# AIGeeksGroup/UniVid

Hardware: AMD Instinct MI355X
Metric: denoise_steps_per_sec (higher is better)
Workload: dtype bf16

## Files before the change

### include/univid_hip.h

```cpp
#ifndef UNIVID_HIP_H
#define UNIVID_HIP_H
#include <stdint.h>
#ifdef __cplusplus
extern "C" {
#endif

int uv_version(void);
const char* uv_build_id(void);
int uv_init(void);
const char* uv_last_error(void);
int uv_device_arch(char* buf, int len);
int uv_host_blocking_sync(int on);

#define UV_OPT_CONV_HALO 0
#define UV_OPT_GEMM_GM 1
#define UV_OPT_ATTN_CUT 2
int uv_set_option(int key, int value);
int uv_get_option(int key, int* value);
int uv_reset_options(void);

#define UV_EPI_BF16 0
#define UV_EPI_GELU_BF16 1
#define UV_EPI_F32_FROM_BF16 2
#define UV_EPI_RESID_F32 3
#define UV_EPI_GATE_RESID_F32 4
#define UV_EPI_BF16_T 5

int uv_gemm_bf16_nt(const void* A, long lda, const void* W, long ldw, const void* bias_bf16, int M, int N, int K,
                    int epilogue, void* out, long ldo, const float* gate, const int32_t* gate_tid, long gate_stride,
                    int tile_cfg, void* stream);

int uv_gemm_bf16_nt_ws(const void* A, long lda, const void* W, long ldw, const void* bias_bf16, int M, int N, int K,
                       int epilogue, void* out, long ldo, const float* gate, const int32_t* gate_tid, long gate_stride,
                       int tile_cfg, void* workspace, long workspace_bytes, void* stream);
long uv_gemm_splitk_ws_bytes(int M, int N, int K);

int uv_gemm_f16_nt(const void* A, long lda, const void* W, long ldw, const void* bias_f16, int M, int N, int K, int epilogue,
                   void* out, long ldo, const float* gate, const int32_t* gate_tid, long gate_stride, int tile_cfg, void* stream);

int uv_gemm_bf16_nt_ssq(const void* A, long lda, const void* W, long ldw, const void* bias_bf16, int M, int N, int K, void* out, long ldo,
                        float* ssq, long ld_ssq, int tile_cfg, void* stream);
int uv_rms_scale_from_ssq(const float* ssq, long ld_ssq, int M, int groups, int C, float eps, float* rs, void* stream);

int uv_lora_down_bf16(const void* x, long ldx, const void* A, long lda, const float* scale, int M, int K, int R, void* out, long ldo,
                      int Rpad, void* stream);


int uv_mx_quant_bf16(const void* x, long ldx, void* codes, long ldc, void* scales, long ld_s, int M, int K, void* stream);

int uv_gemm_mxfp8_nt(const void* A, long lda, const void* A_scale, long ld_as, const void* W, long ldw, const void* W_scale, long ld_ws,
                     const void* bias_bf16, int M, int N, int K, int epilogue, void* out, long ldo, const float* gate,
                     const int32_t* gate_tid, long gate_stride, void* stream);

int uv_gemm_f32_nt(const float* A, long lda, const float* W, long ldw, const float* bias, int M, int N, int K, float* out,
                   long ldo, const float* resid, long ldr, void* stream);

int uv_flash_attn_bf16(const void* q, long ldq, const void* k, long ldk, const void* vt, long ldvt, void* out, long ldo,
                       int batch, int Lq, int Lk, int H, int head_dim, float softmax_scale, void* stream);

int uv_flash_attn_bf16_qnorm(const void* q, long ldq, const void* k, long ldk, const void* vt, long ldvt, void* out, long ldo,
                             int batch, int Lq, int Lk, int H, int head_dim, float softmax_scale, const float* q_rs, const float* q_weight,
                             void* stream);

int uv_flash_attn_f16(const void* q, long ldq, const void* k, long ldk, const void* vt, long ldvt, void* out, long ldo,
                      int batch, int Lq, int Lk, int H, int head_dim, float softmax_scale, void* stream);

int uv_flash_attn_kernel_name(int Lk, int head_dim, long ldk, long ldvt, int f16, char* buf, int len);

// ... 81 lines not shown
```

### univid_amd/_lib.py

```python
import ctypes
import os

import torch

_HERE = os.path.dirname(os.path.abspath(__file__))
LIB_PATH = os.path.join(_HERE, "libunivid_hip.so")

_c = ctypes
_P, _L, _I, _F = _c.c_void_p, _c.c_long, _c.c_int, _c.c_float

SIGNATURES = {
    "uv_version": [],
    "uv_init": [],
    "uv_last_error": [],
    "uv_build_id": [],
    "uv_device_arch": [_c.c_char_p, _I],
    "uv_host_blocking_sync": [_I],
    "uv_set_option": [_I, _I],
    "uv_get_option": [_I, _c.POINTER(_I)],
    "uv_reset_options": [],
    "uv_gemm_bf16_nt": [_P, _L, _P, _L, _P, _I, _I, _I, _I, _P, _L, _P, _P, _L, _I, _P],
    "uv_gemm_bf16_nt_ws": [_P, _L, _P, _L, _P, _I, _I, _I, _I, _P, _L, _P, _P, _L, _I, _P, _L, _P],
    "uv_gemm_splitk_ws_bytes": [_I, _I, _I],
    "uv_gemm_f16_nt": [_P, _L, _P, _L, _P, _I, _I, _I, _I, _P, _L, _P, _P, _L, _I, _P],
    "uv_mx_quant_bf16": [_P, _L, _P, _L, _P, _L, _I, _I, _P],
    "uv_gemm_mxfp8_nt": [_P, _L, _P, _L, _P, _L, _P, _L, _P, _I, _I, _I, _I, _P, _L, _P, _P, _L, _P],
    "uv_gemm_f32_nt": [_P, _L, _P, _L, _P, _I, _I, _I, _P, _L, _P, _L, _P],
    "uv_gemm_bf16_nt_ssq": [_P, _L, _P, _L, _P, _I, _I, _I, _P, _L, _P, _L, _I, _P],
    "uv_rms_scale_from_ssq": [_P, _L, _I, _I, _I, _F, _P, _P],
    "uv_lora_down_bf16": [_P, _L, _P, _L, _P, _I, _I, _I, _P, _L, _I, _P],
    "uv_cast_f32_bf16_rows": [_P, _L, _P, _L, _I, _I, _P],
    "uv_flash_attn_bf16_qnorm": [_P, _L, _P, _L, _P, _L, _P, _L, _I, _I, _I, _I, _I, _F, _P, _P, _P],
    "uv_flash_attn_bf16": [_P, _L, _P, _L, _P, _L, _P, _L, _I, _I, _I, _I, _I, _F, _P],
    "uv_flash_attn_f16": [_P, _L, _P, _L, _P, _L, _P, _L, _I, _I, _I, _I, _I, _F, _P],
    "uv_flash_attn_kernel_name": [_I, _I, _L, _L, _I, _c.c_char_p, _I],
    "uv_flash_attn_plan": [_I, _I, _I, _I, _I, _L, _L, _I, _c.c_char_p, _I, _c.POINTER(_I), _c.POINTER(_I), _c.POINTER(_I)],
    "uv_transpose_16": [_P, _L, _P, _L, _I, _I, _I, _P],
    "uv_cast_f32_to16": [_P, _P, _L, _I, _P],
    "uv_cast_16_to_f32": [_P, _P, _L, _I, _P],
    "uv_layernorm_mod": [_P, _L, _P, _L, _I, _I, _F, _I, _P, _L, _I, _I, _P, _P, _P, _I, _I, _P],
    "uv_t5_attention_bf16": [_P, _L, _P, _L, _P, _L, _P, _L, _I, _I, _P, _I, _P],
    "uv_add_bf16": [_P, _P, _P, _L, _P],
    "uv_t5_gated_gelu_bf16": [_P, _P, _P, _L, _P],
    "uv_gelu_erf_bf16": [_P, _P, _L, _P],
    "uv_interp_linear_rows_bf16": [_P, _L, _P, _L, _I, _I, _I, _P],
    "uv_l2_normalize_rows_f32": [_P, _L, _P, _L, _I, _I, _F, _P],
    "uv_rmsnorm_rope": [_P, _L, _P, _L, _P, _I, _I, _I, _F, _P, _I, _I, _I, _I, _P],
    "uv_rmsnorm_rope_qk": [_P, _P, _P, _P, _P, _P, _L, _L, _I, _I, _I, _I, _F, _P, _I, _I, _I, _I, _P],
    "uv_patchify_bf16": [_P, _P, _L, _I, _I, _I, _I, _I, _I, _I, _I, _P],
    "uv_unpatchify_f32": [_P, _L, _P, _I, _I, _I, _I, _I, _I, _I, _P],
    "uv_sinusoid_f32": [_P, _P, _I, _I, _P],
    "uv_linear_rows_f32": [_P, _L, _P, _P, _P, _L, _I, _I, _I, _I, _P],
    "uv_add_rows_f32": [_P, _P, _P, _I, _L, _P],
    "uv_cast_f32_bf16": [_P, _P, _L, _P],
    "uv_add_bf16_resid": [_P, _L, _P, _L, _I, _I, _P],
    "uv_text_weight_rows_bf16": [_P, _L, _P, _L, _I, _I, _I, _F, _P],
# ... 178 lines not shown
def host_blocking_sync(on=True, device=None):
    dev = torch.device("cuda" if device is None else device)
    idx = torch.cuda.current_device() if dev.index is None else dev.index
    lib = load()
    with torch.cuda.device(idx):
        if lib.uv_host_blocking_sync(1 if on else 0) != 0:
            raise UnividHipError(lib.uv_last_error().decode())


def gemm_splitk_ws_bytes(M, N, K, device=None):
    dev = torch.device("cuda" if device is None else device)
    idx = torch.cuda.current_device() if dev.index is None else dev.index
    lib = init(idx)
    with torch.cuda.device(idx):
        return int(lib.uv_gemm_splitk_ws_bytes(int(M), int(N), int(K)))


def gemm_bf16(a, w, bias, out, epi, M=None, gate=None, gate_tid=None, tile_cfg=0, ws=None):
    f16 = a.dtype == torch.float16
    _chk(a, torch.float16 if f16 else torch.bfloat16, "gemm_bf16.a")
    _chk(w, a.dtype, "gemm_bf16.w")
    M = a.shape[0] if M is None else M
    N, K = w.shape
    if ws is not None and not f16:
        _chk(ws, torch.uint8, "gemm_bf16.ws")
        call("uv_gemm_bf16_nt_ws", ptr(a), a.stride(0), ptr(w), w.stride(0), ptr(bias), M, N, K, epi, ptr(out), out.stride(0),
             ptr(gate), ptr(gate_tid), 0 if gate is None else gate.stride(0), tile_cfg, ptr(ws), ws.numel(), stream_ptr(), flops=2 * M * N * K)
        return out
    call("uv_gemm_f16_nt" if f16 else "uv_gemm_bf16_nt", ptr(a), a.stride(0), ptr(w), w.stride(0), ptr(bias), M, N, K, epi, ptr(out), out.stride(0),
         ptr(gate), ptr(gate_tid), 0 if gate is None else gate.stride(0), tile_cfg, stream_ptr(), flops=2 * M * N * K)
    return out


def mx_quant(x, codes, scales, M=None, K=None):
    _chk(x, torch.bfloat16, "mx_quant.x")
    _chk(codes, torch.uint8, "mx_quant.codes")
    _chk(scales, torch.uint8, "mx_quant.scales")
    M = x.shape[0] if M is None else M
    K = x.shape[1] if K is None else K
    if x.dim() != 2 or codes.dim() != 2 or scales.dim() != 2 or M > min(x.shape[0], codes.shape[0], scales.shape[0]) or \
            K > min(x.shape[1], codes.shape[1]) or K > 32 * scales.shape[1]:
        raise UnividHipError(f"mx_quant: x {tuple(x.shape)} / codes {tuple(codes.shape)} / scales {tuple(scales.shape)} do not fit M = {M}, K = {K}")
    call("uv_mx_quant_bf16", ptr(x), x.stride(0), ptr(codes), codes.stride(0), ptr(scales), scales.stride(0), M, K, stream_ptr())
    return codes, scales


def gemm_mxfp8(a, a_scale, w, w_scale, bias, out, epi, M=None, gate=None, gate_tid=None):
    for t, n in ((a, "a"), (a_scale, "a_scale"), (w, "w"), (w_scale, "w_scale")):
        _chk(t, torch.uint8, "gemm_mxfp8." + n)
    if bias is not None:
        _chk(bias, torch.bfloat16, "gemm_mxfp8.bias")
    M = a.shape[0] if M is None else M
    N, K = w.shape
    if a.shape[1] < K or M > min(a.shape[0], a_scale.shape[0]) or a_scale.shape[1] * 32 < K or w_scale.shape[1] * 32 < K or w_scale.shape[0] < N:
        raise UnividHipError(f"gemm_mxfp8: a {tuple(a.shape)} / a_scale {tuple(a_scale.shape)} / w {tuple(w.shape)} / w_scale "
                             f"{tuple(w_scale.shape)} do not fit M = {M}")
    call("uv_gemm_mxfp8_nt", ptr(a), a.stride(0), ptr(a_scale), a_scale.stride(0), ptr(w), w.stride(0), ptr(w_scale), w_scale.stride(0),
         ptr(bias), M, N, K, epi, ptr(out), out.stride(0), ptr(gate), ptr(gate_tid), 0 if gate is None else gate.stride(0), stream_ptr(),
         flops=2 * M * N * K)
    return out


def gemm_bf16_ssq(a, w, bias, out, ssq, M=None, tile_cfg=0):
    _chk(a, torch.bfloat16, "gemm_bf16_ssq.a")
    _chk(w, torch.bfloat16, "gemm_bf16_ssq.w")
    _chk(ssq, torch.float32, "gemm_bf16_ssq.ssq")
# ... 118 lines not shown
```

### univid_amd/csrc/gemm_bf16.hip

```cpp
#include "gemm_bf16_kernels.h"
#include <limits.h>

int uv_gemm_diag_launch(const GemmArgs& a, int epilogue, int tile_cfg, hipStream_t s);

struct GemmWs { void* p = nullptr; long bytes = 0; };

enum GemmKernel {
    GK_PERSIST,
    GK_PINGPONG,
    GK_RING128,
    GK_T128,
    GK_T256,
    GK_T256x192,
    GK_SPLITK4,
    GK_SPLITK2,
    GK_DIAG,
};
struct GemmStep { GemmKernel kernel; int m0, rows; };
struct GemmPlan { int n; GemmStep step[2]; };

static long whole_rounds_cut(int M, int N, int ncus) {
    const long tiles_n = (N + 255) / 256, tiles_m = (M + 255) / 256;
    const long rounds = tiles_m * tiles_n / ncus;
    return rounds * ncus / tiles_n * 256;
// ... 113 lines not shown
    UV_CHECK_ARG(a.zeros, "uv_gemm_bf16_nt: zero page missing (call uv_init)");
    const GemmPlan plan = plan_gemm(M, N, K, epilogue, ldo, tile_cfg, F16, uv_num_cus(), ws.p ? ws.bytes : 0, ((uintptr_t)ws.p & 255) == 0);
    for (int i = 0; i < plan.n; ++i) {
        const GemmStep& st = plan.step[i];
        const int rc = launch_step<F16>(st.kernel, rows_of(a, epilogue, st.m0, st.rows), epilogue, tile_cfg, (hipStream_t)stream, ws);
        if (rc) return rc;
    }
    return 0;
}

extern "C" int uv_gemm_bf16_nt(const void* A, long lda, const void* W, long ldw, const void* bias_bf16,
                               int M, int N, int K, int epilogue, void* out, long ldo,
                               const float* gate, const int32_t* gate_tid, long gate_stride,
                               int tile_cfg, void* stream) {
    return gemm_entry<false>(A, lda, W, ldw, bias_bf16, M, N, K, epilogue, out, ldo, gate, gate_tid, gate_stride, tile_cfg, stream);
}

extern "C" int uv_gemm_bf16_nt_ws(const void* A, long lda, const void* W, long ldw, const void* bias_bf16,
                                  int M, int N, int K, int epilogue, void* out, long ldo,
                                  const float* gate, const int32_t* gate_tid, long gate_stride,
                                  int tile_cfg, void* workspace, long workspace_bytes, void* stream) {
    UV_CHECK_ARG(workspace_bytes >= 0 && (workspace || workspace_bytes == 0), "uv_gemm_bf16_nt_ws: bad workspace");
    GemmWs ws;
    ws.p = workspace; ws.bytes = workspace_bytes;
    return gemm_entry<false>(A, lda, W, ldw, bias_bf16, M, N, K, epilogue, out, ldo, gate, gate_tid, gate_stride, tile_cfg, stream, nullptr, 0, ws);
}

extern "C" long uv_gemm_splitk_ws_bytes(int M, int N, int K) {
    const GemmPlan plan = plan_gemm(M, N, K, UV_EPI_RESID_F32, N, 0, false, uv_num_cus(), LONG_MAX, true);
    const GemmStep& strip = plan.step[plan.n - 1];
    return strip.kernel == GK_SPLITK4 ? splitk_ws_bytes(strip.rows, N, 4) : 0;
}

extern "C" int uv_gemm_bf16_nt_ssq(const void* A, long lda, const void* W, long ldw, const void* bias_bf16, int M, int N, int K,
                                   void* out, long ldo, float* ssq, long ld_ssq, int tile_cfg, void* stream) {
    return gemm_entry<false>(A, lda, W, ldw, bias_bf16, M, N, K, UV_EPI_BF16_SSQ, out, ldo, nullptr, nullptr, 0, tile_cfg, stream, ssq, ld_ssq);
}

extern "C" int uv_gemm_f16_nt(const void* A, long lda, const void* W, long ldw, const void* bias_f16,
                              int M, int N, int K, int epilogue, void* out, long ldo,
                              const float* gate, const int32_t* gate_tid, long gate_stride,
                              int tile_cfg, void* stream) {
    UV_CHECK_ARG(tile_cfg == 0, "uv_gemm_f16_nt: only tile_cfg 0 (automatic) is built for fp16 operands");
    return gemm_entry<true>(A, lda, W, ldw, bias_f16, M, N, K, epilogue, out, ldo, gate, gate_tid, gate_stride, tile_cfg, stream);
}
```

### univid_amd/csrc/gemm_bf16_kernels.h

```cpp
#pragma once
#include "common.h"
#include <stdlib.h>
#include <type_traits>

const float* uv_zero_page();

#define UV_BK 64

enum {
    UV_EPI_BF16 = 0,
    UV_EPI_GELU_BF16 = 1,
    UV_EPI_F32_FROM_BF16 = 2,
    UV_EPI_RESID_F32 = 3,
    UV_EPI_GATE_RESID_F32 = 4,
    UV_EPI_BF16_T = 5,
    UV_EPI_BF16_SSQ = 6,
};

struct GemmArgs {
    const bf16_t* A;
    const bf16_t* W;
    const bf16_t* bias;
    void* out;
    const float* gate;
// ... 836 lines not shown
            for (int hm = 0; hm < 2; ++hm)
#pragma unroll
                for (int j = 0; j < 4; ++j)
#pragma unroll
                    for (int hn = 0; hn < 2; ++hn)
                        epi_pair16<EPI, F16>(p, m0 + hm * 128 + wr * 64 + j * 16, n0 + hn * 128 + wc * 32, acc[hn][hm][0][j], acc[hn][hm][1][j], frow, fq);
        } else if constexpr (EPI == UV_EPI_BF16_T) {
#pragma unroll
            for (int hm = 0; hm < 2; ++hm)
#pragma unroll
                for (int j = 0; j < 4; j += 2)
#pragma unroll
                    for (int hn = 0; hn < 2; ++hn)
#pragma unroll
                        for (int i = 0; i < 2; ++i)
                            epi_pair16_T<F16>(p, m0 + hm * 128 + wr * 64 + j * 16, n0 + hn * 128 + wc * 32 + i * 16, acc[hn][hm][i][j], acc[hn][hm][i][j + 1], frow, fq);
        } else {
#pragma unroll
            for (int hm = 0; hm < 2; ++hm)
#pragma unroll
                for (int j = 0; j < 4; ++j)
#pragma unroll
                    for (int hn = 0; hn < 2; ++hn)
#pragma unroll
                        for (int i = 0; i < 2; ++i)
                            epi_frag<EPI, F16, true>(p, m0 + hm * 128 + wr * 64 + j * 16, n0 + hn * 128 + wc * 32 + i * 16, acc[hn][hm][i][j], frow, fq);
        }
        if (!has_next) break;
        m0 = m1; n0 = n1; cur = nxt;
    }
    asm volatile("s_waitcnt vmcnt(0)" ::: "memory");
}


template <void (*KERN)(GemmArgs)>
static int launch_kernel(dim3 grid, dim3 block, size_t lds, hipStream_t stream, const GemmArgs& a, const char* who) {
    UV_ONCE_PER_DEVICE(hipFuncSetAttribute((const void*)KERN, hipFuncAttributeMaxDynamicSharedMemorySize, (int)lds));
    hipLaunchKernelGGL(KERN, grid, block, lds, stream, a);
    UV_CHECK_LAUNCH(who);
    return 0;
}

constexpr unsigned UV_EPIS_ALL = 0x7f;
constexpr bool epi_in(unsigned epis, int e) { return e >= 0 && e < 32 && (epis >> e & 1) != 0; }
template <int E>
using epi_c = std::integral_constant<int, E>;
template <unsigned EPIS = UV_EPIS_ALL, class Launch>
static int launch_epi(int epi, Launch&& launch) {
    switch (epi) {
        case UV_EPI_BF16: if constexpr (epi_in(EPIS, UV_EPI_BF16)) return launch(epi_c<UV_EPI_BF16>()); break;
        case UV_EPI_GELU_BF16: if constexpr (epi_in(EPIS, UV_EPI_GELU_BF16)) return launch(epi_c<UV_EPI_GELU_BF16>()); break;
        case UV_EPI_F32_FROM_BF16: if constexpr (epi_in(EPIS, UV_EPI_F32_FROM_BF16)) return launch(epi_c<UV_EPI_F32_FROM_BF16>()); break;
        case UV_EPI_RESID_F32: if constexpr (epi_in(EPIS, UV_EPI_RESID_F32)) return launch(epi_c<UV_EPI_RESID_F32>()); break;
        case UV_EPI_GATE_RESID_F32: if constexpr (epi_in(EPIS, UV_EPI_GATE_RESID_F32)) return launch(epi_c<UV_EPI_GATE_RESID_F32>()); break;
        case UV_EPI_BF16_T: if constexpr (epi_in(EPIS, UV_EPI_BF16_T)) return launch(epi_c<UV_EPI_BF16_T>()); break;
        case UV_EPI_BF16_SSQ: if constexpr (epi_in(EPIS, UV_EPI_BF16_SSQ)) return launch(epi_c<UV_EPI_BF16_SSQ>()); break;
    }
    uv_set_error("uv_gemm_bf16_nt: unknown epilogue %d", epi);
    return -1;
}

template <int VAR = 0, bool F16 = false>
static int launch_8ph(const GemmArgs& a0, int epi, hipStream_t stream) {
    GemmArgs a = a0;
    a.tiles_m = (a.M + 255) / 256;
    a.tiles_n = (a.N + 255) / 256;
// ... 20 lines not shown
                 "uv_gemm_bf16_nt_ws: the split-K strip is built for the bf16 and the residual epilogues (0, 3, 4), not %d", epi);
    a.ws_cnt = (int*)ws;
    a.ws_slab = (float*)((char*)ws + 4096);
    if (hipMemsetAsync(a.ws_cnt, 0, (size_t)tiles * sizeof(int), stream) != hipSuccess) {
        uv_set_error("uv_gemm_bf16_nt_ws: hipMemsetAsync of the tile counters failed");
        return -1;
    }
    const dim3 grid(8 * ((tiles * SK + 7) / 8));
    return launch_epi<EPIS>(epi, [&](auto e) {
        return launch_kernel<gemm_bf16_8ph_kernel<decltype(e)::value, 5, F16, SK>>(grid, 512, 128 * 1024, stream, a, "uv_gemm_bf16_nt_ws");
    });
}

template <bool F16 = false>
static int launch_8ph_persist(const GemmArgs& a0, int epi, hipStream_t stream) {
    GemmArgs a = a0;
    UV_CHECK_ARG(a.M % 256 == 0 && a.N % 256 == 0, "uv_gemm_bf16_nt: the persistent kernel needs whole 256x256 tiles (M=%d N=%d)", a.M, a.N);
    UV_CHECK_ARG(a.ldo % 8 == 0 || (epi != UV_EPI_BF16_T && epi != UV_EPI_BF16 && epi != UV_EPI_GELU_BF16 && epi != UV_EPI_BF16_SSQ),
                 "uv_gemm_bf16_nt: the persistent kernel stores 16 bytes per lane: ldo=%ld must be a multiple of 8 elements", a.ldo);
    a.tiles_m = a.M / 256;
    a.tiles_n = a.N / 256;
    a.gm = (a.N <= 4096 && a.K <= 4096) ? 8 : (a.K >= 8192 ? 2 : 4);
    if (const int gm = uv_option(UV_OPT_GEMM_GM); gm > 0) a.gm = gm;
    const int tiles = a.tiles_m * a.tiles_n;
    int wgs = uv_num_cus() & ~7;
    if (wgs > tiles) wgs = tiles & ~7;
    UV_CHECK_ARG(wgs >= 8, "uv_gemm_bf16_nt: too few tiles (%d) for the persistent kernel", tiles);
    const dim3 grid(wgs);
    return launch_epi(epi, [&](auto e) {
        return launch_kernel<gemm_bf16_8ph_persist_kernel<decltype(e)::value, F16>>(grid, 512, 128 * 1024, stream, a, "uv_gemm_bf16_nt");
    });
}

template <int BM, int BN, int WM, int WN, int NS = 2, bool F16 = false>
static int launch_cfg(const GemmArgs& a0, int epi, hipStream_t stream) {
    GemmArgs a = a0;
    a.tiles_m = (a.M + BM - 1) / BM;
    a.tiles_n = (a.N + BN - 1) / BN;
    constexpr bool SSQ = (BN / WN) % 32 == 0;
    UV_CHECK_ARG(SSQ || epi != UV_EPI_BF16_SSQ, "uv_gemm_bf16_nt_ssq: this tile shape has no whole 32-column groups per wave");
    const dim3 grid(a.tiles_m * a.tiles_n);
    return launch_epi<SSQ ? UV_EPIS_ALL : UV_EPIS_ALL & ~(1u << UV_EPI_BF16_SSQ)>(epi, [&](auto e) {
        return launch_kernel<gemm_bf16_nt_kernel<BM, BN, WM, WN, decltype(e)::value, NS, F16>>(grid, WM * WN * 64, NS * (BM + BN) * 128, stream, a, "uv_gemm_bf16_nt");
    });
}
```

### univid_amd/wan/model.py

```python
import contextlib
import math
from typing import List, Optional

import torch
import torch.nn as nn

from .. import _lib
from .._lib import (EPI_BF16, EPI_BF16_T, EPI_F32_FROM_BF16, EPI_GATE_RESID_F32, EPI_GELU_BF16, EPI_RESID_F32)

__all__ = ["WanModel"]

BF16 = torch.bfloat16


def _round_up(x, m):
    return (x + m - 1) // m * m


def rope_params(max_seq_len, dim, theta=10000):
    ang = torch.outer(torch.arange(max_seq_len),
                      1.0 / torch.pow(theta, torch.arange(0, dim, 2).to(torch.float64).div(dim)))
    return torch.polar(torch.ones_like(ang), ang)


# ... 36 lines not shown
    if mode == "mxfp8":
        if dim % 256 or ffn_dim % 256:
            raise ValueError(f"ffn_precision 'mxfp8' needs dim and ffn_dim to be multiples of 256 (dim {dim}, ffn_dim {ffn_dim}): "
                             "uv_gemm_mxfp8_nt takes N % 256 == 0 and K % 128 == 0")
        if any(getattr(ffn[i], "_uv_lora", None) for i in (0, 2)):
            raise NotImplementedError(
                "ffn_precision 'mxfp8' and an un-merged LoRA adapter (merge=False) on ffn.0 / ffn.2 cannot be combined: the MXFP8 GEMM has no "
                "adapter slot. Detach the adapter or merge it (merge=True: the merged weights are re-quantised), or keep ffn_precision 'bf16'. "
                "Un-merged adapters on the attention projections work in both modes.")


LORA_MAX_SLOT = 512


class _LoraSlot:
    __slots__ = ("A", "scale", "S", "rows")

    def __init__(self, entries, dev):
        self.rows = [(ad, ad["A"].shape[0]) for ad in entries]
        R = sum(r for _, r in self.rows)
        self.S = _round_up(R, 128)
        if self.S > LORA_MAX_SLOT:
            raise ValueError(f"the adapters on the projections of one input stack to rank {R}: more than the {LORA_MAX_SLOT} slot columns "
                             f"(LORA_MAX_SLOT) an activation buffer carries")
        self.A = torch.cat([ad["A"].to(device=dev, dtype=BF16) for ad in entries]).contiguous()
        self.scale = torch.empty(R, dtype=torch.float32, device=dev)
        self.refresh_scale()

    def refresh_scale(self):
        host = torch.cat([torch.full((r,), float(ad["scaling"]) * float(ad["weight"]), dtype=torch.float32) for ad, r in self.rows])
        self.scale.copy_(host)


def _prepare_group(lins):
    preps = {n: _Prepared(l) for n, l in lins.items()}
    entries = [(n, ad) for n, l in lins.items() for ad in getattr(l, "_uv_lora", {}).values()]
    if not entries:
        return preps, None
    first = next(iter(preps.values())).w
    K, dev = first.shape[1], first.device
    slot = _LoraSlot([ad for _, ad in entries], dev)
    col = K
    for n, ad in entries:
        p, r = preps[n], ad["A"].shape[0]
        if p.w.shape[1] == K:
            w = torch.zeros(p.w.shape[0], K + slot.S, dtype=BF16, device=dev)
            w[:, :K] = p.w
            p.w = w
        p.w[:, col:col + r] = ad["B"].to(device=dev, dtype=BF16)
        col += r
    return preps, slot


def _act_buf(rows, K, slots, dev):
    S = max((s.S for s in slots if s is not None), default=0)
    return torch.empty(rows, K + S, dtype=BF16, device=dev)


def _slotted(t, K, slot, M=None):
    if slot is None:
        return t
    M = t.shape[0] if M is None else M
    if t.shape[1] < K + slot.S:
        e = torch.empty(t.shape[0], K + slot.S, dtype=BF16, device=t.device)
        e[:M, :K].copy_(t[:M, :K])
        t = e
    if M:
# ... 2 lines not shown


class WanRMSNorm(nn.Module):
    def __init__(self, dim, eps=1e-5):
        super().__init__()
        self.dim, self.eps = dim, eps
        self.weight = nn.Parameter(torch.ones(dim))


class WanLayerNorm(nn.LayerNorm):
    def __init__(self, dim, eps=1e-6, elementwise_affine=False):
        super().__init__(dim, elementwise_affine=elementwise_affine, eps=eps)


class WanSelfAttention(nn.Module):
    def __init__(self, dim, num_heads, window_size=(-1, -1), qk_norm=True, eps=1e-6):
        assert dim % num_heads == 0
        super().__init__()
        self.dim, self.num_heads, self.head_dim = dim, num_heads, dim // num_heads
        self.window_size, self.qk_norm, self.eps = window_size, qk_norm, eps
        if tuple(window_size) != (-1, -1) or not qk_norm:
            raise NotImplementedError("only the TI2V-5B setting (global attention, qk_norm) is built")
        self.q = nn.Linear(dim, dim)
        self.k = nn.Linear(dim, dim)
        self.v = nn.Linear(dim, dim)
        self.o = nn.Linear(dim, dim)
        self.norm_q = WanRMSNorm(dim, eps=eps)
        self.norm_k = WanRMSNorm(dim, eps=eps)
        self._prep = None
        self._slots = {}
        self._kv_cache = {}

    _groups = {"qkv": ("q", "k", "v"), "o": ("o",)}

    def prepare(self):
        self._prep, self._slots = {}, {}
        for g, names in self._groups.items():
            preps, self._slots[g] = _prepare_group({n: getattr(self, n) for n in names})
            self._prep.update(preps)
        self._kv_cache = {}

    def _self_attn(self, h, L, grid, freqs, x_resid, gate, gate_tid, batch=1, sp=None):
        if sp is not None:
            return self._self_attn_sp(h, L, grid, freqs, x_resid, gate, gate_tid, batch, sp)
        C, H, D = self.dim, self.num_heads, self.head_dim
        p = self._prep
        dev = h.device
        M = batch * L
        h = _slotted(h, C, self._slots["qkv"], M)
        ql = torch.empty(M, C, dtype=BF16, device=dev)
        kl = torch.empty(M, C, dtype=BF16, device=dev)
        vt = _vt_scratch("vt", C, batch, L, dev)
        _lib.gemm_bf16(h, p["q"].w, p["q"].b, ql, EPI_BF16, M=M)
        _lib.gemm_bf16(h, p["k"].w, p["k"].b, kl, EPI_BF16, M=M)
        _lib.gemm_bf16(h, p["v"].w, p["v"].b, vt, EPI_BF16_T, M=M)
        _lib.rmsnorm_rope_qk(ql, kl, self.norm_q.weight, self.norm_k.weight, M, L, C, D, self.eps, freqs, grid)
        att = _act_buf(M, C, (self._slots["o"],), dev)
        _lib.flash_attn(ql, kl, vt, att, L, L, H, D, 1.0 / math.sqrt(D), batch=batch)
        att = _slotted(att, C, self._slots["o"], M)
        _lib.gemm_bf16(att, p["o"].w, p["o"].b, x_resid, EPI_GATE_RESID_F32, M=M, gate=gate, gate_tid=gate_tid)

    def _self_attn_sp(self, h, n, grid, freqs, x_resid, gate, gate_tid, batch, sp):
        par, Lt, r0 = sp
        C, H, D = self.dim, self.num_heads, self.head_dim
        P = par.size
        if H % P or Lt % 8:
            raise NotImplementedError(f"sequence parallel needs heads % ranks == 0 and tokens % 8 == 0 (H={H}, p={P}, L={Lt})")
        p = self._prep
        dev = h.device
        M = batch * n
        Cp, Hp = C // P, H // P
        ql = torch.empty(M, C, dtype=BF16, device=dev)
        kl = torch.empty(M, C, dtype=BF16, device=dev)
        vt = torch.zeros(C, _round_up(max(M, 1), 64), dtype=BF16, device=dev)
        qf = torch.empty(batch * Lt, Cp, dtype=BF16, device=dev)
        kf = torch.empty(batch * Lt, Cp, dtype=BF16, device=dev)
        vtf = _vt_scratch("vt_sp", Cp, batch, Lt, dev)
        if M:
            h = _slotted(h, C, self._slots["qkv"], M)
            _lib.gemm_bf16(h, p["q"].w, p["q"].b, ql, EPI_BF16, M=M)
            _lib.gemm_bf16(h, p["k"].w, p["k"].b, kl, EPI_BF16, M=M)
            _lib.gemm_bf16(h, p["v"].w, p["v"].b, vt, EPI_BF16_T, M=M)
        for b in range(batch):
            rows = slice(b * n, (b + 1) * n)
            if n:
                _lib.rmsnorm_rope(ql[rows], ql[rows], self.norm_q.weight, n, C, D, self.eps, freqs, grid, row0=r0)
                _lib.rmsnorm_rope(kl[rows], kl[rows], self.norm_k.weight, n, C, D, self.eps, freqs, grid, row0=r0)
            par.heads_to_tokens(ql[rows], Lt, qf[b * Lt:(b + 1) * Lt])
            par.heads_to_tokens(kl[rows], Lt, kf[b * Lt:(b + 1) * Lt])
            par.heads_to_tokens_T(vt[:, b * n:(b + 1) * n], Lt, vtf, col0=b * Lt)
        attf = torch.empty(batch * Lt, Cp, dtype=BF16, device=dev)
        _lib.flash_attn(qf, kf, vtf, attf, Lt, Lt, Hp, D, 1.0 / math.sqrt(D), batch=batch)
        att = torch.empty(M, C, dtype=BF16, device=dev)
        for b in range(batch):
            par.tokens_to_heads(attf[b * Lt:(b + 1) * Lt], Lt, att[b * n:(b + 1) * n])
        if M:
            att = _slotted(att, C, self._slots["o"], M)
            _lib.gemm_bf16(att, p["o"].w, p["o"].b, x_resid, EPI_GATE_RESID_F32, M=M, gate=gate, gate_tid=gate_tid)

    def forward(self, x, seq_lens, grid_sizes, freqs):
        _ensure_prepared(self)
        outs = []
        fr = _freqs_device(freqs, x.device)
        for b in range(x.size(0)):
            L = x.size(1)
            Lk = int(seq_lens[b])
            C, H, D = self.dim, self.num_heads, self.head_dim
            p = self._prep
            h = _slotted(x[b].to(BF16).contiguous(), C, self._slots["qkv"])
            ql = torch.empty(L, C, dtype=BF16, device=x.device)
            kl = torch.empty(L, C, dtype=BF16, device=x.device)
            vt = torch.zeros(C, _round_up(L, 64), dtype=BF16, device=x.device)
            _lib.gemm_bf16(h, p["q"].w, p["q"].b, ql, EPI_BF16)
            _lib.gemm_bf16(h, p["k"].w, p["k"].b, kl, EPI_BF16)
            _lib.gemm_bf16(h, p["v"].w, p["v"].b, vt, EPI_BF16_T)
            grid = tuple(int(v) for v in grid_sizes[b])
            _lib.rmsnorm_rope(ql, ql, self.norm_q.weight, L, C, D, self.eps, fr, grid)
            _lib.rmsnorm_rope(kl, kl, self.norm_k.weight, L, C, D, self.eps, fr, grid)
            att = _act_buf(L, C, (self._slots["o"],), x.device)
            _lib.flash_attn(ql, kl, vt, att, L, Lk, H, D, 1.0 / math.sqrt(D))
            att = _slotted(att, C, self._slots["o"])
            y = torch.empty(L, C, dtype=BF16, device=x.device)
            _lib.gemm_bf16(att, p["o"].w, p["o"].b, y, EPI_BF16)
            outs.append(y)
        return torch.stack(outs)


class WanCrossAttention(WanSelfAttention):
    _groups = {"q": ("q",), "kv": ("k", "v"), "o": ("o",)}
    fuse_q_norm = True

    def _context_kv(self, ctx, Lc, batch, kv_key, out=None):
        hit = self._kv_cache.get(kv_key) if kv_key is not None else None
        if hit is not None:
            return hit
        C, D = self.dim, self.head_dim
        p = self._prep
        dev = ctx.device
        ctx = _slotted(ctx, C, self._slots["kv"], batch * Lc)
        if out is not None:
            kl, vt = out
            _lib.gemm_bf16(ctx, p["k"].w, p["k"].b, kl, EPI_BF16, M=batch * Lc)
            _lib.gemm_bf16(ctx, p["v"].w, p["v"].b, vt, EPI_BF16_T, M=batch * Lc)
            _lib.rmsnorm_rope(kl, kl, self.norm_k.weight, batch * Lc, C, D, self.eps)
            return kl, vt
        kl = torch.empty(batch * Lc, C, dtype=BF16, device=dev)
        if kv_key is None:
            vt = _vt_scratch("cvt", C, batch, Lc, dev)
        else:
            if batch > 1 and Lc % 8:
                raise NotImplementedError(f"stacked samples need a context length divisible by 8 (got {Lc})")
            vt = torch.zeros(C, (batch - 1) * Lc + _round_up(Lc, 64), dtype=BF16, device=dev)
        _lib.gemm_bf16(ctx, p["k"].w, p["k"].b, kl, EPI_BF16, M=batch * Lc)
        _lib.gemm_bf16(ctx, p["v"].w, p["v"].b, vt, EPI_BF16_T, M=batch * Lc)
        _lib.rmsnorm_rope(kl, kl, self.norm_k.weight, batch * Lc, C, D, self.eps)
        if kv_key is not None:
            if self._kv_cache and next(iter(self._kv_cache))[0] != kv_key[0]:
                self._kv_cache.clear()
            self._kv_cache[kv_key] = (kl, vt)
        return kl, vt

    def _attend(self, hq, ctx, L, Lc, batch=1, kv_key=None):
# ... 144 lines not shown
            outs.append(xb)
        return torch.stack(outs)


class Head(nn.Module):
    def __init__(self, dim, out_dim, patch_size, eps=1e-6):
        super().__init__()
        self.dim, self.out_dim, self.patch_size, self.eps = dim, out_dim, patch_size, eps
        self.norm = WanLayerNorm(dim, eps)
        self.head = nn.Linear(dim, math.prod(patch_size) * out_dim)
        self.modulation = nn.Parameter(torch.randn(1, 2, dim) / dim ** 0.5)

    def _run(self, x, L, e_rows, tid):
        C = self.dim
        dev = x.device
        n_t = e_rows.shape[0]
        tab = torch.empty(n_t, 2 * C, dtype=torch.float32, device=dev)
        e2 = e_rows.repeat(1, 2).contiguous()
        _lib.call("uv_add_rows_f32", _lib.ptr(self.modulation), _lib.ptr(e2), _lib.ptr(tab), n_t, 2 * C, _lib.stream_ptr())
        hh = torch.empty(L, C, dtype=torch.float32, device=dev)
        _lib.layernorm_mod(x, hh, L, C, self.eps, mode=1, tab=tab, shift_off=0, scale_off=C, tid=tid)
        out = torch.empty(L, self.head.out_features, dtype=torch.float32, device=dev)
        _lib.gemm_f32(hh, self.head.weight, self.head.bias, out, M=L)
        return out


_zero_cache = {}


_ncu = {}


_ws_bytes = {}
SPLITK_STRIP = False


def _splitk_ws_bytes(M, N, K, dev):
    if not SPLITK_STRIP:
        return 0
    key = (M, N, K, str(dev))
    n = _ws_bytes.get(key)
    if n is None:
        n = _ws_bytes[key] = _lib.gemm_splitk_ws_bytes(M, N, K, dev)
    return n


def _ffn0_rows(L, n_cols, dev):
    Lp = _round_up(L, 256)
    if Lp == L or n_cols % 256:
        return L
    ncu = _ncu.get(dev)
    if ncu is None:
        ncu = _ncu[dev] = max(8, torch.cuda.get_device_properties(dev).multi_processor_count & ~7)
    tn = n_cols // 256
    full, padded = (L // 256) * tn, (Lp // 256) * tn
    return Lp if full >= 2 * ncu and -(-padded // ncu) == -(-full // ncu) else L


def _zeros_cached(key, shape, dtype, device):
    t = _zero_cache.get(key)
    if t is None or tuple(t.shape) != tuple(shape) or (t.is_inference() and not torch.is_inference_mode_enabled()):
        t = torch.zeros(shape, dtype=dtype, device=device)
        _zero_cache[key] = t
    return t


# ... 326 lines not shown
```

Measured before the change: 3.971.

## Fuse Q/K/V projections into one grouped persistent GEMM launch

Stacks the q, k and v weights (and biases) into one contiguous matrix and adds a grouped persistent GEMM kernel. A single launch walks the combined N tiles, and each tile's epilogue routes to the right output, including the transposed V layout. The intent is to remove two kernel launches and the partial tail wave of each small GEMM, while reusing A tiles across the projections. A planner compares the grouped tile rounds against the sum of per-projection rounds and falls back to three separate GEMMs when grouping does not help. Risks include a fixed tile shape without the split-K or strip variants, and per-tile member and transpose branching in the epilogue.

```diff
diff --git a/include/univid_hip.h b/include/univid_hip.h
--- a/include/univid_hip.h
+++ b/include/univid_hip.h
@@ -34,6 +34,10 @@
                        int epilogue, void* out, long ldo, const float* gate, const int32_t* gate_tid, long gate_stride,
                        int tile_cfg, void* workspace, long workspace_bytes, void* stream);
 long uv_gemm_splitk_ws_bytes(int M, int N, int K);
+
+int uv_gemm_bf16_nt_group(const void* A, long lda, long a_rows, const void* W, long ldw, const void* bias_bf16, int M, int K, int n_proj,
+                          const int* N, const int* epilogue, void* const* out, const long* ldo, int tile_cfg, void* stream);
+int uv_gemm_group_plan(int M, long a_rows, int K, int n_proj, const int* N, const int* epilogue, const long* ldo, int tile_cfg, int ncus);
 
 int uv_gemm_f16_nt(const void* A, long lda, const void* W, long ldw, const void* bias_f16, int M, int N, int K, int epilogue,
                    void* out, long ldo, const float* gate, const int32_t* gate_tid, long gate_stride, int tile_cfg, void* stream);
diff --git a/univid_amd/_lib.py b/univid_amd/_lib.py
--- a/univid_amd/_lib.py
+++ b/univid_amd/_lib.py
@@ -22,6 +22,8 @@
     "uv_gemm_bf16_nt": [_P, _L, _P, _L, _P, _I, _I, _I, _I, _P, _L, _P, _P, _L, _I, _P],
     "uv_gemm_bf16_nt_ws": [_P, _L, _P, _L, _P, _I, _I, _I, _I, _P, _L, _P, _P, _L, _I, _P, _L, _P],
     "uv_gemm_splitk_ws_bytes": [_I, _I, _I],
+    "uv_gemm_bf16_nt_group": [_P, _L, _L, _P, _L, _P, _I, _I, _I, _c.POINTER(_I), _c.POINTER(_I), _c.POINTER(_P), _c.POINTER(_L), _I, _P],
+    "uv_gemm_group_plan": [_I, _L, _I, _I, _c.POINTER(_I), _c.POINTER(_I), _c.POINTER(_L), _I, _I],
     "uv_gemm_f16_nt": [_P, _L, _P, _L, _P, _I, _I, _I, _I, _P, _L, _P, _P, _L, _I, _P],
     "uv_mx_quant_bf16": [_P, _L, _P, _L, _P, _L, _I, _I, _P],
     "uv_gemm_mxfp8_nt": [_P, _L, _P, _L, _P, _L, _P, _L, _P, _I, _I, _I, _I, _P, _L, _P, _P, _L, _P],
@@ -266,6 +268,37 @@
     return out
 
 
+def gemm_bf16_group(a, w, bias, outs, epis, M=None, a_rows=None, tile_cfg=0):
+    _chk(a, torch.bfloat16, "gemm_bf16_group.a")
+    _chk(w, torch.bfloat16, "gemm_bf16_group.w")
+    n = len(outs)
+    if n != len(epis) or not 1 <= n <= 4:
+        raise UnividHipError(f"gemm_bf16_group: 1 .. 4 outputs with one epilogue each (got {n} / {len(epis)})")
+    for o in outs:
+        _chk(o, torch.bfloat16, "gemm_bf16_group.out")
+    M = a.shape[0] if M is None else M
+    a_rows = a.shape[0] if a_rows is None else a_rows
+    K = w.shape[1]
+    Ns = [o.shape[0] if e == EPI_BF16_T else o.shape[1] for o, e in zip(outs, epis)]
+    if sum(Ns) != w.shape[0] or (bias is not None and bias.numel() != w.shape[0]):
+        raise UnividHipError(f"gemm_bf16_group: the outputs' columns {Ns} do not add up to the {w.shape[0]} rows of w (and bias)")
+    first = ptr(outs[0])
+    for o in outs[1:]:
+        if ptr(o).dev != first.dev:
+            raise UnividHipError("gemm_bf16_group: outputs must live on ONE GPU")
+    call("uv_gemm_bf16_nt_group", ptr(a), a.stride(0), a_rows, ptr(w), w.stride(0), ptr(bias), M, K, n, (_I * n)(*Ns), (_I * n)(*epis),
+         (_P * n)(*[o.data_ptr() for o in outs]), (_L * n)(*[o.stride(0) for o in outs]), tile_cfg, stream_ptr(), flops=2 * M * sum(Ns) * K)
+    return outs
+
+
+def gemm_group_plan(M, a_rows, K, Ns, epis, ldos, tile_cfg=0, ncus=0):
+    n = len(Ns)
+    rc = load().uv_gemm_group_plan(int(M), int(a_rows), int(K), n, (_I * n)(*Ns), (_I * n)(*epis), (_L * n)(*ldos), int(tile_cfg), int(ncus))
+    if rc < 0:
+        raise UnividHipError(load().uv_last_error().decode())
+    return rc
+
+
 def mx_quant(x, codes, scales, M=None, K=None):
     _chk(x, torch.bfloat16, "mx_quant.x")
     _chk(codes, torch.uint8, "mx_quant.codes")
diff --git a/univid_amd/csrc/gemm_bf16.hip b/univid_amd/csrc/gemm_bf16.hip
--- a/univid_amd/csrc/gemm_bf16.hip
+++ b/univid_amd/csrc/gemm_bf16.hip
@@ -169,6 +169,98 @@
     return strip.kernel == GK_SPLITK4 ? splitk_ws_bytes(strip.rows, N, 4) : 0;
 }
 
+
+static constexpr double GROUP_STRIP_ROUNDS = 0.48;
+
+struct GroupPlan { bool grouped; long rounds; };
+
+static GroupPlan plan_gemm_group(int M, long a_rows, int K, int n_proj, const int* N, const int* epilogue, const long* ldo, int tile_cfg,
+                                 int ncus) {
+    if ((tile_cfg != 0 && tile_cfg != 17) || n_proj < 1 || n_proj > UV_GROUP_MAX || M <= 0) return {false, 0};
+    if (K % 128 != 0 || K < 384) return {false, 0};
+    const long Mp = ((long)M + 255) / 256 * 256;
+    if (a_rows < Mp) return {false, 0};
+    long tiles_n = 0;
+    for (int i = 0; i < n_proj; ++i) {
+        if (N[i] <= 0 || N[i] % 256 != 0 || ldo[i] % 8 != 0) return {false, 0};
+        if (epilogue[i] != UV_EPI_BF16 && epilogue[i] != UV_EPI_BF16_T) return {false, 0};
+        if (epilogue[i] == UV_EPI_BF16_T && M % 8 != 0) return {false, 0};
+        tiles_n += N[i] / 256;
+    }
+    const long tiles = Mp / 256 * tiles_n;
+    if (tiles < 8 || tiles_n > 254) return {false, 0};
+    const long rounds = (tiles + ncus - 1) / ncus;
+    if (tile_cfg == 17) return {true, rounds};
+    double own = 0;
+    for (int i = 0; i < n_proj; ++i) {
+        const GemmPlan pl = plan_gemm(M, N[i], K, epilogue[i], ldo[i], 0, false, ncus, 0, false);
+        const GemmStep& main = pl.step[0];
+        if (main.kernel != GK_PERSIST && main.kernel != GK_PINGPONG) return {false, rounds};
+        own += (double)(((long)(main.rows + 255) / 256 * (N[i] / 256) + ncus - 1) / ncus) + (pl.n == 2 ? GROUP_STRIP_ROUNDS : 0.0);
+    }
+    return {(double)rounds < own, rounds};
+}
+
+extern "C" int uv_gemm_group_plan(int M, long a_rows, int K, int n_proj, const int* N, const int* epilogue, const long* ldo, int tile_cfg,
+                                  int ncus) {
+    UV_CHECK_ARG(N && epilogue && ldo && n_proj >= 1 && n_proj <= UV_GROUP_MAX, "uv_gemm_group_plan: 1 .. %d members with N, epilogue and ldo", UV_GROUP_MAX);
+    const GroupPlan g = plan_gemm_group(M, a_rows, K, n_proj, N, epilogue, ldo, tile_cfg, ncus > 0 ? ncus : uv_num_cus());
+    return g.grouped ? (int)g.rounds : 0;
+}
+
+extern "C" int uv_gemm_bf16_nt_group(const void* A, long lda, long a_rows, const void* W, long ldw, const void* bias_bf16, int M, int K,
+                                     int n_proj, const int* N, const int* epilogue, void* const* out, const long* ldo, int tile_cfg,
+                                     void* stream) {
+    UV_CHECK_ARG(A && W && N && epilogue && out && ldo, "uv_gemm_bf16_nt_group: null pointer");
+    UV_CHECK_ARG(n_proj >= 1 && n_proj <= UV_GROUP_MAX, "uv_gemm_bf16_nt_group: 1 .. %d projections (got %d)", UV_GROUP_MAX, n_proj);
+    UV_CHECK_ARG(M > 0 && K > 0 && a_rows >= M, "uv_gemm_bf16_nt_group: bad shape M=%d K=%d a_rows=%ld", M, K, a_rows);
+    for (int i = 0; i < n_proj; ++i) {
+        UV_CHECK_ARG(out[i] && N[i] > 0, "uv_gemm_bf16_nt_group: projection %d: null output or N=%d", i, N[i]);
+        UV_CHECK_ARG(epilogue[i] == UV_EPI_BF16 || epilogue[i] == UV_EPI_BF16_T,
+                     "uv_gemm_bf16_nt_group: projection %d: epilogue %d (only UV_EPI_BF16 and UV_EPI_BF16_T)", i, epilogue[i]);
+    }
+    const GroupPlan g = plan_gemm_group(M, a_rows, K, n_proj, N, epilogue, ldo, tile_cfg, uv_num_cus());
+    if (!g.grouped) {
+        UV_CHECK_ARG(tile_cfg != 17, "uv_gemm_bf16_nt_group: tile_cfg 17 (the grouped launch) needs N_i %% 256 == 0, K %% 128 == 0, K >= 384, "
+                     "ldo_i %% 8 == 0, a_rows >= M rounded up to 256, M %% 8 == 0 with a transposed output, and at least 8 tiles");
+        long n0 = 0;
+        for (int i = 0; i < n_proj; ++i) {
+            const int rc = gemm_entry<false>(A, lda, (const bf16_t*)W + n0 * ldw, ldw, bias_bf16 ? (const bf16_t*)bias_bf16 + n0 : nullptr, M, N[i], K,
+                                             epilogue[i], out[i], ldo[i], nullptr, nullptr, 0, tile_cfg, stream);
+            if (rc) return rc;
+            n0 += N[i];
+        }
+        return 0;
+    }
+    UV_CHECK_ARG(lda % 8 == 0 && ldw % 8 == 0, "uv_gemm_bf16_nt_group: lda/ldw must be multiples of 8 elements");
+    UV_CHECK_ARG(((uintptr_t)A & 15) == 0 && ((uintptr_t)W & 15) == 0 && ((uintptr_t)bias_bf16 & 7) == 0,
+                 "uv_gemm_bf16_nt_group: A and W must be 16-byte aligned, bias 8-byte aligned");
+    UV_CHECK_ARG(lda >= K && ldw >= K, "uv_gemm_bf16_nt_group: lda=%ld / ldw=%ld below K=%d", lda, ldw, K);
+    GemmGroupArgs a;
+    a.A = (const bf16_t*)A; a.W = (const bf16_t*)W; a.bias = (const bf16_t*)bias_bf16;
+    a.lda = lda; a.ldw = ldw; a.M = M; a.K = K; a.n_proj = n_proj; a.gm = 0;
+    a.zeros = uv_zero_page();
+    UV_CHECK_ARG(a.zeros, "uv_gemm_bf16_nt_group: zero page missing (call uv_init)");
+    a.tiles_m = (M + 255) / 256;
+    UV_CHECK_ARG(lda < (1L << 22) && ldw < (1L << 22), "uv_gemm_bf16_nt_group: lda=%ld / ldw=%ld: the kernel's lane offsets take 256 rows in 32 bits", lda, ldw);
+    int tn = 0;
+    a.tile_end = 0; a.trans = 0;
+    for (int i = 0; i < UV_GROUP_MAX; ++i) {
+        const bool live = i < n_proj;
+        if (live) {
+            UV_CHECK_ARG(((uintptr_t)out[i] & 15) == 0, "uv_gemm_bf16_nt_group: projection %d: output must be 16-byte aligned", i);
+            UV_CHECK_ARG(ldo[i] >= (epilogue[i] == UV_EPI_BF16_T ? M : N[i]) && ldo[i] < (1L << 23), "uv_gemm_bf16_nt_group: projection %d: ldo=%ld too small (or 2^23 and above)", i, ldo[i]);
+            tn += N[i] / 256;
+            if (epilogue[i] == UV_EPI_BF16_T) a.trans |= 1 << i;
+        }
+        a.tile_end |= (uint32_t)(i + 1 < n_proj ? tn : 255) << (8 * i);
+        a.out[i] = live ? (bf16_t*)out[i] : nullptr;
+        a.ldo[i] = live ? (int)ldo[i] : 0;
+    }
+    a.tiles_n = tn;
+    return launch_8ph_group<false>(a, (hipStream_t)stream);
+}
+
 extern "C" int uv_gemm_bf16_nt_ssq(const void* A, long lda, const void* W, long ldw, const void* bias_bf16, int M, int N, int K,
                                    void* out, long ldo, float* ssq, long ld_ssq, int tile_cfg, void* stream) {
     return gemm_entry<false>(A, lda, W, ldw, bias_bf16, M, N, K, UV_EPI_BF16_SSQ, out, ldo, nullptr, nullptr, 0, tile_cfg, stream, ssq, ld_ssq);
diff --git a/univid_amd/csrc/gemm_bf16_kernels.h b/univid_amd/csrc/gemm_bf16_kernels.h
--- a/univid_amd/csrc/gemm_bf16_kernels.h
+++ b/univid_amd/csrc/gemm_bf16_kernels.h
@@ -892,6 +892,194 @@
     asm volatile("s_waitcnt vmcnt(0)" ::: "memory");
 }
 
+#define UV_GROUP_MAX 4
+struct GemmGroupArgs {
+    const bf16_t* A;
+    const bf16_t* W;
+    const bf16_t* bias;
+    const float* zeros;
+    long lda, ldw;
+    int M, K;
+    int tiles_m, tiles_n;
+    int gm;
+    int n_proj;
+    uint32_t tile_end;
+    int trans;
+    bf16_t* out[UV_GROUP_MAX];
+    int ldo[UV_GROUP_MAX];
+};
+
+template <bool ROWBIAS, bool MASK, bool F16>
+__device__ __forceinline__ void epi_pair16_group(bf16_t* o, int ldo, const bf16_t* bias, int rows, int cols, int mb, int nb,
+                                                 const f32x4& a0, const f32x4& a1, int frow, int fq) {
+    const int m = mb + frow;
+    uint32_t w[2][2];
+    if (ROWBIAS) {
+        const float b = in16<F16>(bias[m]);
+        w[0][0] = pack16_2<F16>(a0[0] + b, a0[1] + b); w[0][1] = pack16_2<F16>(a0[2] + b, a0[3] + b);
+        w[1][0] = pack16_2<F16>(a1[0] + b, a1[1] + b); w[1][1] = pack16_2<F16>(a1[2] + b, a1[3] + b);
+    } else {
+#pragma unroll
+        for (int f = 0; f < 2; ++f) {
+            const u32x2 bb = *(const u32x2*)(bias + nb + 16 * f + 4 * fq);
+            const f32x4& a = f ? a1 : a0;
+            w[f][0] = pack16_2<F16>(a[0] + in16<F16>((bf16_t)(bb[0] & 0xffff)), a[1] + in16<F16>((bf16_t)(bb[0] >> 16)));
+            w[f][1] = pack16_2<F16>(a[2] + in16<F16>((bf16_t)(bb[1] & 0xffff)), a[3] + in16<F16>((bf16_t)(bb[1] >> 16)));
+        }
+    }
+    const auto s0 = __builtin_amdgcn_permlane16_swap(w[0][0], w[1][0], false, false);
+    const auto s1 = __builtin_amdgcn_permlane16_swap(w[0][1], w[1][1], false, false);
+    const u32x4 v = {(uint32_t)s0[0], (uint32_t)s1[0], (uint32_t)s0[1], (uint32_t)s1[1]};
+    const int col = nb + ((fq & 1) << 4) + ((fq >> 1) << 3);
+    if (!MASK || (m < rows && col < cols)) *(u32x4*)(o + (uint32_t)(m * ldo + col)) = v;
+}
+
+template <bool ROWBIAS, bool MASK, bool F16>
+__device__ __forceinline__ void epi_tile_group(bf16_t* o, int ldo, const bf16_t* bias, int rows, int cols, const f32x4 (&acc)[2][2][2][4],
+                                               int wr, int wc, int frow, int fq) {
+#pragma unroll
+    for (int hm = 0; hm < 2; ++hm)
+#pragma unroll
+        for (int j = 0; j < 4; ++j)
+#pragma unroll
+            for (int hn = 0; hn < 2; ++hn)
+                epi_pair16_group<ROWBIAS, MASK, F16>(o, ldo, bias, rows, cols, hm * 128 + wr * 64 + j * 16, hn * 128 + wc * 32,
+                                                     acc[hn][hm][0][j], acc[hn][hm][1][j], frow, fq);
+}
+
+template <bool F16 = false>
+__global__ __launch_bounds__(512) void gemm_bf16_8ph_group_kernel(GemmGroupArgs p) {
+    constexpr bool TRANS = false;
+    constexpr int VAR = 5;
+    constexpr int HALF = 16384;
+    constexpr int BUF = 4 * HALF;
+    extern __shared__ __attribute__((aligned(16))) char smem[];
+
+    const int tid = threadIdx.x;
+    const int lane = tid & 63;
+    const int wave = __builtin_amdgcn_readfirstlane(tid >> 6);
+    const int wr = wave >> 2, wc = wave & 3;
+
+    const int nblk = p.tiles_m * p.tiles_n;
+    const int G = gridDim.x >> 3;
+    int first, cnt;
+    {
+        const int q = nblk >> 3, r = nblk & 7, xcd = blockIdx.x & 7;
+        first = xcd < r ? xcd * (q + 1) : r * (q + 1) + (xcd - r) * q;
+        cnt = q + (xcd < r ? 1 : 0);
+    }
+    int cur = blockIdx.x >> 3;
+    if (cur >= cnt) return;
+    const int GM = p.gm;
+    const int group_sz = GM * p.tiles_n;
+    auto origin = [&](int bid, int& m0, int& n0) {
+        const int group = bid / group_sz;
+        const int first_m = group * GM;
+        const int gm = min(GM, p.tiles_m - first_m);
+        const int in_group = bid - group * group_sz;
+        m0 = (first_m + in_group % gm) * 256;
+        n0 = (in_group / gm) * 256;
+    };
+    auto member = [&](int tn) {
+        return (tn >= (int)(p.tile_end & 255) ? 1 : 0) + (tn >= (int)(p.tile_end >> 8 & 255) ? 1 : 0) + (tn >= (int)(p.tile_end >> 16 & 255) ? 1 : 0);
+    };
+    int m0, n0;
+    origin(first + cur, m0, n0);
+
+    auto lane_off = [&](long ld) {
+        int t = tid;
+        asm volatile("" : "+v"(t));
+        const int srow8 = t >> 3;
+        return srow8 * (int)ld + (((t & 7) ^ ((srow8 >> 1) & 7)) << 3);
+    };
+    const bf16_t* a_src[2][2];
+    const bf16_t* w_src[2][2];
+    auto set_a = [&](int h, int m, int n, bool tr) {
+        const long ld = tr ? p.ldw : p.lda;
+        const bf16_t* base = (tr ? p.W + (long)n * ld : p.A + (long)m * ld) + h * 128 * ld;
+        const int off = lane_off(ld);
+        a_src[h][0] = base + off;
+        a_src[h][1] = base + 64 * ld + off;
+    };
+    auto set_w = [&](int h, int m, int n, bool tr) {
+        const long ld = tr ? p.lda : p.ldw;
+        const bf16_t* base = (tr ? p.A + (long)m * ld : p.W + (long)n * ld) + h * 128 * ld;
+        const int off = lane_off(ld);
+        w_src[h][0] = base + off;
+        w_src[h][1] = base + 64 * ld + off;
+    };
+    int r0 = member(n0 >> 8);
+    {
+        const bool tr = (p.trans >> r0 & 1) != 0;
+        set_a(0, m0, n0, tr); set_a(1, m0, n0, tr); set_w(0, m0, n0, tr); set_w(1, m0, n0, tr);
+    }
+    char* const my_dst = smem + wave * 1024;
+    const int nk = p.K / UV_BK;
+    const int frow = lane & 15, fq = lane >> 4;
+    const int lx = (fq ^ (frow >> 1)) << 4;
+    const char* const la = smem + (wr * 64 + frow) * 128;
+    const char* const lw = smem + 2 * HALF + (wc * 32 + frow) * 128;
+    f32x4 acc[2][2][2][4];
+    bf16x8 af[4][2], w0[2][2], w1[2][2];
+
+    UV_STAGE(w_src[0], 0, 2 * HALF) UV_STAGE(w_src[1], 0, 3 * HALF) UV_STAGE(a_src[0], 0, 0) UV_STAGE(a_src[1], 0, HALF)
+    UV_STAGE(w_src[1], 1, BUF + 3 * HALF) UV_STAGE(a_src[0], 1, BUF)
+    asm volatile("s_waitcnt vmcnt(6)" ::: "memory");
+    UV_SB();
+    for (;;) {
+        if (wr == 1) UV_SB();
+#pragma unroll
+        for (int a = 0; a < 2; ++a)
+#pragma unroll
+            for (int b = 0; b < 2; ++b)
+#pragma unroll
+                for (int i = 0; i < 2; ++i)
+#pragma unroll
+                    for (int j = 0; j < 4; ++j) acc[a][b][i][j] = (f32x4){0.f, 0.f, 0.f, 0.f};
+
+        const int nxt = cur + G;
+        const bool has_next = nxt < cnt;
+        int m1 = m0, n1 = n0;
+        if (has_next) origin(first + nxt, m1, n1);
+        const int r1 = member(n1 >> 8);
+        const bool tr1 = (p.trans >> r1 & 1) != 0;
+        int t = 0;
+        for (; t + 2 < nk; t += 2) {
+            UV_KTILE5(t, 0, 1, true, true)
+            UV_KTILE5(t + 1, 1, 0, true, true)
+        }
+        set_w(1, m1, n1, tr1); set_a(0, m1, n1, tr1);
+        UV_KTILE5X(nk - 1, 0, 0, 1, true, true)
+        set_w(0, m1, n1, tr1);
+        set_a(1, m1, n1, tr1);
+        UV_KTILE5X(0, 1, 1, 0, true, true)
+        if (wr == 0) UV_SB();
+
+        {
+            const int r = r0;
+            bf16_t* const out = p.out[r];
+            const int ldo = p.ldo[r];
+            const bool trans = (p.trans >> r & 1) != 0;
+            const int tn0 = r ? (int)(p.tile_end >> (8 * (r - 1)) & 255) : 0;
+            const int nloc = n0 - tn0 * 256;
+            const bf16_t* const bias = p.bias ? p.bias + n0 : (const bf16_t*)p.zeros;
+            const int live = p.M - m0;
+            if (!trans) {
+                bf16_t* const o = out + (long)m0 * ldo + nloc;
+                if (live >= 256) epi_tile_group<false, false, F16>(o, ldo, bias, 256, 256, acc, wr, wc, frow, fq);
+                else epi_tile_group<false, true, F16>(o, ldo, bias, live, 256, acc, wr, wc, frow, fq);
+            } else {
+                bf16_t* const o = out + (long)nloc * ldo + m0;
+                if (live >= 256) epi_tile_group<true, false, F16>(o, ldo, bias, 256, 256, acc, wr, wc, frow, fq);
+                else epi_tile_group<true, true, F16>(o, ldo, bias, 256, live, acc, wr, wc, frow, fq);
+            }
+        }
+        if (!has_next) break;
+        m0 = m1; n0 = n1; cur = nxt; r0 = r1;
+    }
+    asm volatile("s_waitcnt vmcnt(0)" ::: "memory");
+}
+
 
 template <void (*KERN)(GemmArgs)>
 static int launch_kernel(dim3 grid, dim3 block, size_t lds, hipStream_t stream, const GemmArgs& a, const char* who) {
@@ -978,6 +1166,21 @@
     });
 }
 
+template <bool F16 = false>
+static int launch_8ph_group(const GemmGroupArgs& a0, hipStream_t stream) {
+    GemmGroupArgs a = a0;
+    a.gm = a.K <= 4096 ? 8 : (a.K >= 8192 ? 2 : 4);
+    if (const int gm = uv_option(UV_OPT_GEMM_GM); gm > 0) a.gm = gm;
+    const int tiles = a.tiles_m * a.tiles_n;
+    int wgs = uv_num_cus() & ~7;
+    if (wgs > tiles) wgs = tiles & ~7;
+    UV_CHECK_ARG(wgs >= 8, "uv_gemm_bf16_nt_group: too few tiles (%d) for the persistent kernel", tiles);
+    UV_ONCE_PER_DEVICE(hipFuncSetAttribute((const void*)gemm_bf16_8ph_group_kernel<F16>, hipFuncAttributeMaxDynamicSharedMemorySize, 128 * 1024));
+    hipLaunchKernelGGL(gemm_bf16_8ph_group_kernel<F16>, dim3(wgs), 512, 128 * 1024, stream, a);
+    UV_CHECK_LAUNCH("uv_gemm_bf16_nt_group");
+    return 0;
+}
+
 template <int BM, int BN, int WM, int WN, int NS = 2, bool F16 = false>
 static int launch_cfg(const GemmArgs& a0, int epi, hipStream_t stream) {
     GemmArgs a = a0;
diff --git a/univid_amd/wan/model.py b/univid_amd/wan/model.py
--- a/univid_amd/wan/model.py
+++ b/univid_amd/wan/model.py
@@ -92,7 +92,43 @@
         self.scale.copy_(host)
 
 
-def _prepare_group(lins):
+def _rows_allocated(t):
+    have = t.untyped_storage().nbytes() // t.element_size() - t.storage_offset()
+    return 0 if have < t.shape[1] else (have - t.shape[1]) // t.stride(0) + 1
+
+
+class _Stacked:
+    __slots__ = ("w", "b")
+
+    def __init__(self, w, b):
+        self.w, self.b = w, b
+
+
+def _stack_group(preps, stack):
+    members = list(preps.values())
+    Kw = max(m.w.shape[1] for m in members)
+    with_b = [m.b is not None for m in members]
+    if any(with_b) != all(with_b):
+        return
+    w = torch.cat([m.w if m.w.shape[1] == Kw else torch.nn.functional.pad(m.w, (0, Kw - m.w.shape[1])) for m in members])
+    b = torch.cat([m.b for m in members]) if all(with_b) else None
+    r = 0
+    for m in members:
+        n = m.w.shape[0]
+        m.w = w[r:r + n]
+        m.b = None if b is None else b[r:r + n]
+        r += n
+    preps[stack] = _Stacked(w, b)
+
+
+def _prepare_group(lins, stack=None):
+    preps, slot = _prepare_members(lins)
+    if stack is not None:
+        _stack_group(preps, stack)
+    return preps, slot
+
+
+def _prepare_members(lins):
     preps = {n: _Prepared(l) for n, l in lins.items()}
     entries = [(n, ad) for n, l in lins.items() for ad in getattr(l, "_uv_lora", {}).values()]
     if not entries:
@@ -161,13 +197,26 @@
         self._kv_cache = {}
 
     _groups = {"qkv": ("q", "k", "v"), "o": ("o",)}
+    _stacked = ("qkv",)
 
     def prepare(self):
         self._prep, self._slots = {}, {}
         for g, names in self._groups.items():
-            preps, self._slots[g] = _prepare_group({n: getattr(self, n) for n in names})
+            preps, self._slots[g] = _prepare_group({n: getattr(self, n) for n in names}, stack=g if g in self._stacked else None)
             self._prep.update(preps)
         self._kv_cache = {}
+
+    def _qkv(self, h, M, ql, kl, vt):
+        p = self._prep
+        C = self.dim
+        h = _slotted(h, C, self._slots["qkv"], M)
+        if QKV_GROUP and "qkv" in p:
+            rows = max(h.shape[0], _rows_allocated(h))
+            _lib.gemm_bf16_group(h, p["qkv"].w, p["qkv"].b, (ql, kl, vt), (EPI_BF16, EPI_BF16, EPI_BF16_T), M=M, a_rows=rows)
+            return
+        _lib.gemm_bf16(h, p["q"].w, p["q"].b, ql, EPI_BF16, M=M)
+        _lib.gemm_bf16(h, p["k"].w, p["k"].b, kl, EPI_BF16, M=M)
+        _lib.gemm_bf16(h, p["v"].w, p["v"].b, vt, EPI_BF16_T, M=M)
 
     def _self_attn(self, h, L, grid, freqs, x_resid, gate, gate_tid, batch=1, sp=None):
         if sp is not None:
@@ -176,13 +225,10 @@
         p = self._prep
         dev = h.device
         M = batch * L
-        h = _slotted(h, C, self._slots["qkv"], M)
         ql = torch.empty(M, C, dtype=BF16, device=dev)
         kl = torch.empty(M, C, dtype=BF16, device=dev)
         vt = _vt_scratch("vt", C, batch, L, dev)
-        _lib.gemm_bf16(h, p["q"].w, p["q"].b, ql, EPI_BF16, M=M)
-        _lib.gemm_bf16(h, p["k"].w, p["k"].b, kl, EPI_BF16, M=M)
-        _lib.gemm_bf16(h, p["v"].w, p["v"].b, vt, EPI_BF16_T, M=M)
+        self._qkv(h, M, ql, kl, vt)
         _lib.rmsnorm_rope_qk(ql, kl, self.norm_q.weight, self.norm_k.weight, M, L, C, D, self.eps, freqs, grid)
         att = _act_buf(M, C, (self._slots["o"],), dev)
         _lib.flash_attn(ql, kl, vt, att, L, L, H, D, 1.0 / math.sqrt(D), batch=batch)
@@ -206,10 +252,7 @@
         kf = torch.empty(batch * Lt, Cp, dtype=BF16, device=dev)
         vtf = _vt_scratch("vt_sp", Cp, batch, Lt, dev)
         if M:
-            h = _slotted(h, C, self._slots["qkv"], M)
-            _lib.gemm_bf16(h, p["q"].w, p["q"].b, ql, EPI_BF16, M=M)
-            _lib.gemm_bf16(h, p["k"].w, p["k"].b, kl, EPI_BF16, M=M)
-            _lib.gemm_bf16(h, p["v"].w, p["v"].b, vt, EPI_BF16_T, M=M)
+            self._qkv(h, M, ql, kl, vt)
         for b in range(batch):
             rows = slice(b * n, (b + 1) * n)
             if n:
@@ -257,6 +300,7 @@
 
 class WanCrossAttention(WanSelfAttention):
     _groups = {"q": ("q",), "kv": ("k", "v"), "o": ("o",)}
+    _stacked = ()
     fuse_q_norm = True
 
     def _context_kv(self, ctx, Lc, batch, kv_key, out=None):
@@ -467,6 +511,7 @@
 
 
 _ws_bytes = {}
+QKV_GROUP = True
 SPLITK_STRIP = False
 
 
```

New measurement: 3.979, median of 6. No clear change (+0.2%).
